# FrankVeenstra/gym_rem2D

Hardware: AMD Instinct MI355X
Metric: env steps/sec (whole node) at 65 536 parallel creatures; 1/2/4/8-GPU scaling (higher is better)
Workload: dtype f32

## Files before the change

### gym_rem2d_amd/csrc/rem2d_vel4.h

```cpp
#ifndef REM2D_VEL4_H
#define REM2D_VEL4_H

#ifndef V4_PLUS1_GAIN
#define V4_PLUS1_GAIN 2
#endif
#ifndef V4_PHASES
#ifdef REM2D_WIDE
#define V4_PHASES 5
#else
#define V4_PHASES 4
#endif
#endif
#define V4_MAX_BODIES 256
#define V4_MAX_PASSES (V4_MAX_BODIES / WAVE)

struct Vel4Args { int velIters; float dt; int prio, prioT1, prioT2;  int dbg;  };
#ifdef REM2D_V4_PROBES
#define V4_DBG(A) ((A).dbg)
#else
#define V4_DBG(A) 0

#endif

struct __attribute__((aligned(16))) V4Vel { float x, y, w, invI; };
template <int SETS, int PASSES> struct Vel4Shared {
    V4Vel vel[PASSES * WAVE];
    unsigned short jmap[SETS][WAVE];
    unsigned int cmap[PASSES * WAVE * KT];
    int firstR[PASSES * WAVE], lastR[PASSES * WAVE];
    unsigned glmap[PASSES * WAVE];
};

struct JointT {
    V2 rA, rB;
    float mA, mB;
    float exx, eyx, eyy, motorMass, det33, det22;
    float ezx, ezy, cyzx, cyzy, cyzz;
    float impX, impY, impZ, motorImp, motorSpeed, maxMotorImpulse;
    int key;
};
#define V4_JA(k) ((k) & 0xff)
#define V4_JB(k) (((k) >> 8) & 0xff)
#define V4_JROUND(k) (((k) >> 16) & 0xff)
#define V4_LIMIT(k) (((k) >> 24) & 0x3)
#define V4_JPHASE(k) (((k) >> 26) & 0x7)
#define V4_VALID(k) ((k) < 0)

DEV void v4_joint_load(const State &S, const unsigned *glmap, int K, int child, float h, int P, int rotation, JointT &J) {
    const unsigned Lp = S.Lp;
    const unsigned gl = glmap[child];
    const int jA = (child & ~(K - 1)) + LI(L_PARENT);
    const int jround = (LI(L_JROUND) & 0xff) + rotation;
    const unsigned jb = (unsigned)SCR_JREC_BASE * Lp + gl;
    J.rA = mk(SW(jb, 0), SW(jb, 1));
    J.rB = mk(SW(jb, 2), SW(jb, 3));
    J.mB = LF(L_INVM);
    const float iB = LF(L_INVI);
    J.impX = LF(L_JIMPX); J.impY = LF(L_JIMPY); J.impZ = LF(L_JIMPZ); J.motorImp = LF(L_JMOTORIMP);
    J.motorSpeed = LF(L_JMOTORSPEED);
    const int limitState = LI(L_JLIMIT);
    J.maxMotorImpulse = h * LF(L_JTORQUE);
    float iA;
    {
        const unsigned gl = glmap[jA];
        J.mA = LF(L_INVM); iA = LF(L_INVI);
    }
    J.key = jA | (child << 8) | (jround << 16) | (limitState << 24) | ((jround % P) << 26) | (int)0x80000000;
    const float mA = J.mA, mB = J.mB;
    const V2 rA = J.rA, rB = J.rB;
    J.exx = mA + mB + rA.y * rA.y * iA + rB.y * rB.y * iB;
    J.eyx = -rA.y * rA.x * iA - rB.y * rB.x * iB;
    const float ezx = -rA.y * iA - rB.y * iB;
    J.eyy = mA + mB + rA.x * rA.x * iA + rB.x * rB.x * iB;
    const float ezy = rA.x * iA + rB.x * iB;
    const float ezz = iA + iB;
    J.motorMass = iA + iB;
    if (J.motorMass > 0.0f) J.motorMass = 1.0f / J.motorMass;
    const float cyzx = J.eyy * ezz - ezy * ezy;
    const float cyzy = ezy * ezx - J.eyx * ezz;
    const float cyzz = J.eyx * ezy - J.eyy * ezx;
    J.ezx = ezx; J.ezy = ezy; J.cyzx = cyzx; J.cyzy = cyzy; J.cyzz = cyzz;
    J.det33 = J.exx * cyzx + J.eyx * cyzy + ezx * cyzz;
    if (J.det33 != 0.0f) J.det33 = 1.0f / J.det33;
    J.det22 = J.exx * J.eyy - J.eyx * J.eyx;
    if (J.det22 != 0.0f) J.det22 = 1.0f / J.det22;
}

template <typename SH> DEV void v4_joint_slot(JointT &j, SH &sh) {
    const int a = V4_JA(j.key), b = V4_JB(j.key), limitState = V4_LIMIT(j.key);
    V4Vel ra = sh.vel[a], rb = sh.vel[b];
    V2 vA = mk(ra.x, ra.y), vB = mk(rb.x, rb.y);
    float wA = ra.w, wB = rb.w;
    const float iA = ra.invI, iB = rb.invI;
    if (limitState != LIM_EQUAL) {
        float Cdot = wB - wA - j.motorSpeed;
        float impulse = -j.motorMass * Cdot;
        float oldImpulse = j.motorImp;
        j.motorImp = fclamp(oldImpulse + impulse, -j.maxMotorImpulse, j.maxMotorImpulse);
        impulse = j.motorImp - oldImpulse;
        wA -= iA * impulse;
        wB += iB * impulse;
    }
    const V2 Cdot1 = vsub(vsub(vadd(vB, vcross_sv(wB, j.rB)), vA), vcross_sv(wA, j.rA));
    float ix, iy, iz = 0.0f;
    if (limitState != LIM_INACTIVE) {
        const float ezx = j.ezx, ezy = j.ezy, ezz = iA + iB;
        const float cyzx = j.cyzx, cyzy = j.cyzy, cyzz = j.cyzz;
        float Cdot2 = wB - wA;
        float bx = Cdot1.x, by = Cdot1.y, bz = Cdot2;
        float sx = j.det33 * (bx * cyzx + by * cyzy + bz * cyzz);
        float cbx = by * ezz - bz * ezy, cby = bz * ezx - bx * ezz, cbz = bx * ezy - by * ezx;
        float sy = j.det33 * (j.exx * cbx + j.eyx * cby + ezx * cbz);
        float ebx = j.eyy * bz - ezy * by, eby = ezy * bx - j.eyx * bz, ebz = j.eyx * by - j.eyy * bx;
        float sz = j.det33 * (j.exx * ebx + j.eyx * eby + ezx * ebz);
        ix = -sx; iy = -sy; iz = -sz;
        if (limitState == LIM_EQUAL) {
            j.impX += ix; j.impY += iy; j.impZ += iz;
        } else {
            float newImpulse = j.impZ + iz;
            bool reduce = (limitState == LIM_AT_LOWER ? newImpulse : -newImpulse) < 0.0f;
            if (reduce) {
                V2 rhs = vadd(vneg(Cdot1), vscale(j.impZ, mk(ezx, ezy)));
                float rx = j.det22 * (j.eyy * rhs.x - j.eyx * rhs.y);
                float ry = j.det22 * (j.exx * rhs.y - j.eyx * rhs.x);
                ix = rx; iy = ry; iz = -j.impZ;
                j.impX += rx; j.impY += ry; j.impZ = 0.0f;
            } else {
                j.impX += ix; j.impY += iy; j.impZ += iz;
            }
        }
    } else {
        V2 bb = vneg(Cdot1);
        ix = j.det22 * (j.eyy * bb.x - j.eyx * bb.y);
        iy = j.det22 * (j.exx * bb.y - j.eyx * bb.x);
        j.impX += ix; j.impY += iy;
    }
    {
        V2 P = mk(ix, iy);
        vA = vsub(vA, vscale(j.mA, P));
        wA -= iA * (vcross(j.rA, P) + iz);
        vB = vadd(vB, vscale(j.mB, P));
        wB += iB * (vcross(j.rB, P) + iz);
    }
    ra.x = vA.x; ra.y = vA.y; ra.w = wA;
    rb.x = vB.x; rb.y = vB.y; rb.w = wB;
    sh.vel[a] = ra;
    sh.vel[b] = rb;
}

struct ContactT {
    ContactC c;
    QuadRole r;
    float mB;
    int key;
};
#define V4_CBODY(k) ((k) & 0xff)
#define V4_CSUB(k) (((k) >> 8) & 0xf)
#define V4_CT(k) (((k) >> 12) & 0xf)
static_assert(KT <= 16, "manifold index: 4 bits");
#define V4_COFF(k) (((k) >> 16) & 0xff)
#define V4_CPHASE(k) (((k) >> 24) & 0x7)

template <int CSETS, bool CPAIR, typename SH>
DEV void v4_contact_subslots(const State &S, ContactT (&C)[CSETS], SH &sh, int lane, int NC, bool spill,
                             bool pair, int nsub, int ph, int tick, int span, float mu) {
    const unsigned Lp = S.Lp;
    for (int t = 0; t < nsub; ++t) {
#pragma unroll
        for (int cs = 0; cs < CSETS; ++cs) {
            if (V4_VALID(C[cs].key) && V4_CSUB(C[cs].key) == t && V4_CPHASE(C[cs].key) == ph &&
                (unsigned)(tick - V4_COFF(C[cs].key)) < (unsigned)span) {
                const int b = V4_CBODY(C[cs].key);
                V4Vel v = sh.vel[b];
                if (!CPAIR || !pair) {
                    contact_solve(C[cs].c, C[cs].mB, v.invI, mu, v.x, v.y, v.w);
                    sh.vel[b] = v;
                } else {
                    float vq = C[cs].r.isY ? v.y : v.x;
                    contact_solve_pair(C[cs].c, C[cs].r, C[cs].mB, v.invI, mu, vq, v.w);
                    if (!C[cs].r.isY) sh.vel[b].x = vq;
                    else { sh.vel[b].y = vq; sh.vel[b].w = v.w; }
                }
            }
        }
        if (spill) {
            for (int ci = CSETS * WAVE + lane; ci < NC; ci += WAVE) {
                const int e = (int)sh.cmap[ci];
                const int b = V4_CBODY(e);
                if (V4_CSUB(e) != t || V4_CPHASE(e) != ph || !((unsigned)(tick - V4_COFF(e)) < (unsigned)span)) continue;
                const unsigned gl = sh.glmap[b];
                const unsigned cb = (unsigned)(SCR_CC_BASE + V4_CT(e) * CC_WORDS) * Lp + gl;
                ContactC c;
                cc_load(S, cb, c);
                V4Vel v = sh.vel[b];
                contact_solve(c, LF(L_INVM), v.invI, mu, v.x, v.y, v.w);
                sh.vel[b] = v;
                SW(cb, 10) = c.n0; SW(cb, 11) = c.n1; SW(cb, 12) = c.t0; SW(cb, 13) = c.t1;
            }
        }
        lds_sync();
    }
}

template <int SETS, int PASSES, int CSETS, bool CPAIR, bool FLEXP = true>
DEV void vel4_body(const State &S, const float friction, const Vel4Args &A, unsigned tile, int K, Vel4Shared<SETS, PASSES> &sh) {
    const int lane = threadIdx.x;
    const unsigned Lp = S.Lp;
    constexpr bool FLEX = FLEXP && SETS <= 3;
    const int c0 = S.tiles[tile], c1 = S.tiles[tile + 1];
    const int NB = (c1 - c0) * K;
    const unsigned long long rEntry = (V4_DBG(A) & (16 | 64)) ? __builtin_amdgcn_s_memrealtime() : 0;
    const bool retile = FLEX && (S.flags & (REM2D_FLAG_RETILE | REM2D_STATE_ORDERED)) != 0;
    const int iters = A.velIters;
    const float h = A.dt, mu = friction;
    const unsigned long long below = lane == 0 ? 0ull : (~0ull >> (WAVE - lane));
    if (S.flags & REM2D_FLAG_SKIP_FROZEN) {
        bool allSkipped = true;
        for (int e = c0 + lane; e < c1; e += WAVE) {
            const unsigned env = retile ? (unsigned)S.order[e] : (unsigned)e;
            const int m0 = __float_as_int(SW((unsigned)SCR_MISC_BASE * Lp + env * (unsigned)K, 0));
            allSkipped = allSkipped && (m0 & 0x200) != 0;
        }
        if (__all(allSkipped ? 1 : 0)) return;
    }

#pragma unroll
    for (int s = 0; s < SETS; ++s) sh.jmap[s][lane] = 0xffff;
    int sched[PASSES], misc[PASSES], parent[PASSES];
    int P = 1;
#pragma unroll
    for (int p = 0; p < PASSES; ++p) {
        const int bl = p * WAVE + lane;
        const unsigned ce = (unsigned)c0 + (unsigned)(bl / K);
        const unsigned gl = ((retile && bl < NB) ? (unsigned)S.order[ce] : ce) * (unsigned)K + (unsigned)(bl & (K - 1));
        sh.glmap[bl] = gl;
        sched[p] = 0; misc[p] = 0; parent[p] = -1;
        sh.firstR[bl] = 0x7fffffff;
        sh.lastR[bl] = -1;
        if (bl < NB) {
            misc[p] = __float_as_int(SW((unsigned)SCR_MISC_BASE * Lp + gl, 0));
            sched[p] = LI(L_JROUND);
            parent[p] = LI(L_PARENT);
            V4Vel v;
            v.x = LF(L_VX); v.y = LF(L_VY); v.w = LF(L_W); v.invI = LF(L_INVI);
            sh.vel[bl] = v;
        }
        P = max(P, (sched[p] >> 16) & 0xff);
    }
    P = wave_max(P);
    lds_sync();
#pragma unroll
    for (int p = 0; p < PASSES; ++p) {
        const int bl = p * WAVE + lane;
        if ((misc[p] & 0x100) != 0 && parent[p] >= 0) {
            const int jr = sched[p] & 0xff, pl = (bl & ~(K - 1)) + parent[p];
            atomicMin(&sh.firstR[bl], jr); atomicMax(&sh.lastR[bl], jr);
            atomicMin(&sh.firstR[pl], jr); atomicMax(&sh.lastR[pl], jr);
        }
    }
    lds_sync();
    const unsigned long long groupLanes = (K >= WAVE ? ~0ull : ((1ull << K) - 1ull)) << (lane & ~(K - 1) & (WAVE - 1));
    int offB[PASSES], delta[PASSES];
    auto plan = [&](const int Pc) -> int {
        int wlo[PASSES], wlen[PASSES];
        bool placed[PASSES];
#pragma unroll
        for (int p = 0; p < PASSES; ++p) {
            const int bl = p * WAVE + lane;
            const bool solve = (misc[p] & 0x100) != 0;
            const int nT = solve ? (misc[p] & 0xff) : 0;
            const int lastB = sh.lastR[bl];
            wlo[p] = lastB >= 0 ? lastB : 0;
            wlen[p] = lastB >= 0 ? sh.firstR[bl] + Pc - lastB : Pc;
            offB[p] = wlo[p];
            placed[p] = nT == 0;
            delta[p] = 0;
        }
        int subs[V4_PHASES];
#pragma unroll
        for (int s = 0; s < V4_PHASES; ++s) subs[s] = 0;
#pragma unroll
        for (int p = 0; p < PASSES; ++p) {
            const int wl = wlo[p] % Pc;
            for (int round = 0; round < Pc && round < V4_PHASES; ++round) {
                int cover[V4_PHASES];
#pragma unroll
                for (int s = 0; s < V4_PHASES; ++s) {
                    int d = s - wl;
                    d = d < 0 ? d + Pc : d;
                    cover[s] = __popcll(__ballot(!placed[p] && s < Pc && d < wlen[p]) & groupLanes);
                }
                int cstar = 0;
#pragma unroll
                for (int s = 1; s < V4_PHASES; ++s) cstar = (s < Pc && cover[s] >= cover[cstar]) ? s : cstar;
                int dstar = cstar - wl;
                dstar = dstar < 0 ? dstar + Pc : dstar;
                if (!placed[p] && cover[cstar] > 0 && dstar < wlen[p]) {
                    offB[p] = wlo[p] + dstar;
                    placed[p] = true;
                }
            }
            const bool solve = (misc[p] & 0x100) != 0;
            const int nT = solve ? (misc[p] & 0xff) : 0;
            if (FLEX) {
                const int cph = offB[p] % Pc;
                int heavyPhase = 0, heavy = 0;
#pragma unroll
                for (int s = 0; s < V4_PHASES; ++s) {
                    int most = 0;
#pragma unroll
                    for (int n = 1; n <= KT; ++n) most = (__ballot(nT >= n && cph == s) & groupLanes) ? n : most;
                    if (s < Pc && most > heavy) { heavy = most; heavyPhase = s; }
                }
                delta[p] = heavy > 0 ? (Pc - heavyPhase) % Pc : 0;
            }
            const int cphr = (offB[p] + delta[p]) % Pc;
#pragma unroll
            for (int s = 0; s < V4_PHASES; ++s) {
#pragma unroll
                for (int n = 1; n <= KT; ++n)
                    if (__ballot(nT >= n && cphr == s)) subs[s] = max(subs[s], n);
            }
        }
        int total = 0;
#pragma unroll
        for (int s = 0; s < V4_PHASES; ++s) total += subs[s];
        return total;
    };
    {
        const int subsP = plan(P);
        if (FLEX && P < V4_PHASES && subsP >= 3) {
            int offP[PASSES], deltaP[PASSES];
#pragma unroll
            for (int p = 0; p < PASSES; ++p) { offP[p] = offB[p]; deltaP[p] = delta[p]; }
            const int subsQ = plan(P + 1);
            if (subsQ + V4_PLUS1_GAIN <= subsP) P = P + 1;
            else {
#pragma unroll
                for (int p = 0; p < PASSES; ++p) { offB[p] = offP[p]; delta[p] = deltaP[p]; }
            }
        }
    }
#pragma unroll
    for (int p = 0; p < PASSES; ++p) sh.firstR[p * WAVE + lane] = delta[p];
    lds_sync();

    int NC = 0, lastTick = -1, maxRound = -1, err = 0, maxT = 0;
    int jcount[SETS];
#pragma unroll
    for (int s = 0; s < SETS; ++s) jcount[s] = 0;
    int subMax[V4_PHASES];
#pragma unroll
    for (int s = 0; s < V4_PHASES; ++s) subMax[s] = 0;
#pragma unroll
    for (int p = 0; p < PASSES; ++p) {
        const int bl = p * WAVE + lane;
        const bool solve = (misc[p] & 0x100) != 0;
        const bool hasJ = solve && parent[p] >= 0;
        const int nT = solve ? (misc[p] & 0xff) : 0;
        const int jr = (sched[p] & 0xff) + delta[p];
        const int phase = jr % P;
        if (!FLEX) {
#pragma unroll
            for (int s = 0; s < SETS; ++s) {
                const unsigned long long m = __ballot(hasJ && phase % SETS == s);
                if (hasJ && phase % SETS == s) {
                    const int rank = jcount[s] + __popcll(m & below);
                    if (rank < WAVE) sh.jmap[s][rank] = (unsigned short)bl;
                    else err = REM2D_ERR_SOLVER_OVERFLOW;
                }
                jcount[s] += __popcll(m);
            }
        } else {
            bool placedJ = !hasJ;
#pragma unroll
            for (int k = 0; k < SETS; ++k) {
#pragma unroll
                for (int s = 0; s < SETS; ++s) {
                    const bool want = !placedJ && (phase + k) % SETS == s;
                    const unsigned long long m = __ballot(want);
                    if (want) {
                        const int rank = jcount[s] + __popcll(m & below);
                        if (rank < WAVE) { sh.jmap[s][rank] = (unsigned short)bl; placedJ = true; }
                    }
                    jcount[s] = min(WAVE, jcount[s] + __popcll(m));
                }
            }
            if (!placedJ) err = REM2D_ERR_SOLVER_OVERFLOW;
        }
        if (hasJ && phase >= V4_PHASES) err = REM2D_ERR_SOLVER_OVERFLOW;
        const int off = offB[p] + delta[p];
        const int cph = off % P;
        if (nT > 0) {
#pragma unroll
            for (int s = 0; s < V4_PHASES; ++s)
                if (cph == s) subMax[s] = max(subMax[s], nT);
            if (cph >= V4_PHASES) err = REM2D_ERR_SOLVER_OVERFLOW;
            if (iters > 0) lastTick = max(lastTick, off + (iters - 1) * P);
        }
#pragma unroll
        for (int t = 0; t < KT; ++t) {
            const unsigned long long cm = __ballot(nT > t);
            if (nT > t) sh.cmap[NC + __popcll(cm & below)] = (unsigned)(bl | (t << 8) | (t << 12) | (off << 16) | (cph << 24));
            NC += __popcll(cm);
        }
        maxT = max(maxT, nT);
        if (iters > 0 && hasJ) lastTick = max(lastTick, jr + (iters - 1) * P);
        if (hasJ) maxRound = max(maxRound, jr);
    }
    const int nTicks = wave_max(lastTick) + 1;
    const int nRounds = wave_max(maxRound) + 1;
    maxT = wave_max(maxT);
#pragma unroll
    for (int s = 0; s < V4_PHASES; ++s) subMax[s] = (V4_DBG(A) & 1) ? 0 : wave_max(subMax[s]);
    lds_sync();
    if (A.prio & 1) {
        int cost = 7 * P;
#pragma unroll
        for (int s = 0; s < V4_PHASES; ++s) cost += 10 * subMax[s];
        if (cost >= A.prioT2) __builtin_amdgcn_s_setprio(3);
        else if (cost >= A.prioT1) __builtin_amdgcn_s_setprio(1);
    }

    JointT J[SETS];
#pragma unroll
    for (int s = 0; s < SETS; ++s) {
        J[s].key = 0;
        const int child = sh.jmap[s][lane];
        if (child != 0xffff) v4_joint_load(S, sh.glmap, K, child, h, P, sh.firstR[child], J[s]);
    }
    ContactT C[CSETS];
    const bool pair = CPAIR && NC <= CSETS * (WAVE / 2);
#pragma unroll
    for (int cs = 0; cs < CSETS; ++cs) {
        C[cs].key = 0;
        C[cs].c.count = 0;
        C[cs].mB = 0.0f;
        C[cs].r.tq = C[cs].r.nq = C[cs].r.r0c = C[cs].r.r1c = 0.0f;
        C[cs].r.isY = (lane & 1) != 0;
        C[cs].r.pt1 = false;
        const int ci = pair ? cs * (WAVE / 2) + (lane >> 1) : cs * WAVE + lane;
        if (ci < NC) {
            const int e = (int)sh.cmap[ci];
            const int b = V4_CBODY(e), t = V4_CT(e);
            const unsigned gl = sh.glmap[b];
            C[cs].key = e | (int)0x80000000;
            C[cs].mB = LF(L_INVM);
            cc_load(S, (unsigned)(SCR_CC_BASE + t * CC_WORDS) * Lp + gl, C[cs].c);
            C[cs].r = quad_role(C[cs].c, lane);
        }
    }
    const int CCAP = CSETS * WAVE;
    const bool spill = NC > CCAP;
    for (int t = 0; t < maxT; ++t) {
#pragma unroll
        for (int cs = 0; cs < CSETS; ++cs) {
            if (V4_VALID(C[cs].key) && V4_CT(C[cs].key) == t) {
                const int b = V4_CBODY(C[cs].key);
                V4Vel v = sh.vel[b];
                contact_warm_start(C[cs].c, C[cs].mB, v.invI, v.x, v.y, v.w);
                sh.vel[b] = v;
            }
        }
        if (spill) {
            for (int ci = CCAP + lane; ci < NC; ci += WAVE) {
                const int e = (int)sh.cmap[ci];
                const int b = V4_CBODY(e);
                if (V4_CT(e) != t) continue;
                const unsigned gl = sh.glmap[b];
                ContactC c;
                cc_load(S, (unsigned)(SCR_CC_BASE + t * CC_WORDS) * Lp + gl, c);
                V4Vel v = sh.vel[b];
                contact_warm_start(c, LF(L_INVM), v.invI, v.x, v.y, v.w);
                sh.vel[b] = v;
            }
        }
        lds_sync();
    }
    for (int r = 0; r < nRounds; ++r) {
#pragma unroll
        for (int s = 0; s < SETS; ++s) {
            if (V4_VALID(J[s].key) && V4_JROUND(J[s].key) == r) {
                const int a = V4_JA(J[s].key), b = V4_JB(J[s].key);
                V4Vel ra = sh.vel[a], rb = sh.vel[b];
                V2 vA = mk(ra.x, ra.y), vB = mk(rb.x, rb.y);
                float wA = ra.w, wB = rb.w;
                V2 Pw = mk(J[s].impX, J[s].impY);
                vA = vsub(vA, vscale(J[s].mA, Pw));
                wA -= ra.invI * (vcross(J[s].rA, Pw) + J[s].motorImp + J[s].impZ);
                vB = vadd(vB, vscale(J[s].mB, Pw));
                wB += rb.invI * (vcross(J[s].rB, Pw) + J[s].motorImp + J[s].impZ);
                ra.x = vA.x; ra.y = vA.y; ra.w = wA;
                rb.x = vB.x; rb.y = vB.y; rb.w = wB;
                sh.vel[a] = ra;
                sh.vel[b] = rb;
            }
        }
        lds_sync();
    }
    {
        const int span = iters * P;
        const bool joints = !(V4_DBG(A) & 2);
        const bool stamp = (V4_DBG(A) & (8 | 32)) != 0;
        unsigned long long tJ = 0, tC = 0, t0 = 0, t1 = 0, nSub = 0;
        const unsigned long long tStart = stamp ? __builtin_amdgcn_s_memtime() : 0;
        const unsigned long long rStart = stamp ? __builtin_amdgcn_s_memrealtime() : 0;
        for (int base = 0; base < nTicks; base += P) {
#pragma unroll
            for (int s = 0; s < V4_PHASES; ++s) {
                if (s < P) {
                    const int tick = base + s;
                    if (stamp) t0 = __builtin_amdgcn_s_memtime();
                    {
                        JointT &Js = J[s % SETS];
                        if (joints && V4_VALID(Js.key) && (SETS == V4_PHASES || V4_JPHASE(Js.key) == s) &&
                            (unsigned)(tick - V4_JROUND(Js.key)) < (unsigned)span) v4_joint_slot(Js, sh);
                    }
                    if (FLEX && SETS > 1) {
#pragma unroll
                        for (int q = 1; q < SETS; ++q) {
                            JointT &Jo = J[(s + q) % SETS];
                            if (joints && V4_VALID(Jo.key) && V4_JPHASE(Jo.key) == s &&
                                (unsigned)(tick - V4_JROUND(Jo.key)) < (unsigned)span) v4_joint_slot(Jo, sh);
                        }
                    }
                    lds_sync();
                    if (stamp) { t1 = __builtin_amdgcn_s_memtime(); tJ += t1 - t0; }
                    v4_contact_subslots<CSETS, CPAIR>(S, C, sh, lane, NC, spill, pair, subMax[s], s, tick, span, mu);
                    if (stamp) { tC += __builtin_amdgcn_s_memtime() - t1; nSub += subMax[s]; }
                }
            }
        }
        if ((V4_DBG(A) & 32) && lane == 0 && c1 - c0 >= 4) {
            const unsigned long long tAll = __builtin_amdgcn_s_memtime() - tStart;
            unsigned env = (unsigned)c0;
            EI(E_TOIEVENTS) = (int)(tJ >> 6);
            env = (unsigned)c0 + 1; EI(E_TOIEVENTS) = (int)(tC >> 6);
            env = (unsigned)c0 + 2; EI(E_TOIEVENTS) = (int)(tAll >> 6);
            env = (unsigned)c0 + 3; EI(E_TOIEVENTS) = (int)((nSub << 16) | (unsigned long long)(nTicks & 0xffff));
        }
        if ((V4_DBG(A) & 8) && lane == 0 && c1 - c0 >= 5) {
            const unsigned long long tAll = __builtin_amdgcn_s_memtime() - tStart;
            unsigned env = (unsigned)c0;
            EI(E_TOIEVENTS) = (int)(tJ >> 4);
            env = (unsigned)c0 + 1; EI(E_TOIEVENTS) = (int)(tC >> 4);
            env = (unsigned)c0 + 2; EI(E_TOIEVENTS) = (int)(tAll >> 4);
            env = (unsigned)c0 + 3; EI(E_TOIEVENTS) = (int)nSub;
            env = (unsigned)c0 + 4; EI(E_TOIEVENTS) = nTicks;
            if (c1 - c0 >= 6) { env = (unsigned)c0 + 5; EI(E_TOIEVENTS) = (int)(__builtin_amdgcn_s_memrealtime() - rStart); }
        }
    }
#pragma unroll
    for (int cs = 0; cs < CSETS; ++cs) {
        if (V4_VALID(C[cs].key) && !(pair && (lane & 1))) {
            const int b = V4_CBODY(C[cs].key), t = V4_CT(C[cs].key);
            const unsigned gl = sh.glmap[b];
            const slotpack_t sp = sp_load(S, (unsigned)SCR_MISC_BASE * Lp + gl);
            const unsigned o = SP_GET(sp, t) * Lp + gl;
            CF(C_N0, o) = C[cs].c.n0;
            CF(C_T0, o) = C[cs].c.t0;
            if (C[cs].c.count > 1) {
                CF(C_N1, o) = C[cs].c.n1;
                CF(C_T1, o) = C[cs].c.t1;
            }
        }
    }
    if (spill) {
        for (int ci = CCAP + lane; ci < NC; ci += WAVE) {
            const int e = (int)sh.cmap[ci];
            const int b = V4_CBODY(e), t = V4_CT(e);
            const unsigned gl = sh.glmap[b];
            const unsigned cb = (unsigned)(SCR_CC_BASE + t * CC_WORDS) * Lp + gl;
            const slotpack_t sp = sp_load(S, (unsigned)SCR_MISC_BASE * Lp + gl);
            const unsigned o = SP_GET(sp, t) * Lp + gl;
            CF(C_N0, o) = SW(cb, 10);
            CF(C_T0, o) = SW(cb, 12);
            if (__float_as_int(SW(cb, 20)) > 1) {
                CF(C_N1, o) = SW(cb, 11);
                CF(C_T1, o) = SW(cb, 13);
            }
        }
    }
#pragma unroll
    for (int s = 0; s < SETS; ++s) {
        if (V4_VALID(J[s].key)) {
            const unsigned gl = sh.glmap[V4_JB(J[s].key)];
            LF(L_JIMPX) = J[s].impX; LF(L_JIMPY) = J[s].impY; LF(L_JIMPZ) = J[s].impZ; LF(L_JMOTORIMP) = J[s].motorImp;
        }
    }
#pragma unroll
    for (int p = 0; p < PASSES; ++p) {
        const int bl = p * WAVE + lane;
        if (misc[p] & 0x100) {
            const unsigned gl = sh.glmap[bl];
            const V4Vel v = sh.vel[bl];
            LF(L_VX) = v.x; LF(L_VY) = v.y; LF(L_W) = v.w;
        }
    }
    err = wave_or(err);
    if (err) {
        for (int e = c0 + lane; e < c1; e += WAVE) {
            const unsigned env = retile ? (unsigned)S.order[e] : (unsigned)e;
            atomicOr(&EI(E_ERR), err);
        }
    }
    if ((V4_DBG(A) & 64) && lane == 0) {
        const unsigned env = (unsigned)c0;
        EI(E_TOIEVENTS) = (int)(__builtin_amdgcn_s_memrealtime() - rEntry);
    }
    if ((V4_DBG(A) & 16) && lane == 0 && c1 - c0 >= 2) {
        unsigned env = (unsigned)c0;
        EI(E_TOIEVENTS) = (int)(rEntry & 0x7fffffff);
        env = (unsigned)c0 + 1; EI(E_TOIEVENTS) = (int)(__builtin_amdgcn_s_memrealtime() & 0x7fffffff);
    }
}

struct Vel4Batch {
    State S[REM2D_MAX_BATCH];
    float friction[REM2D_MAX_BATCH];
    unsigned tileEnd[REM2D_MAX_BATCH];
    int lanes[REM2D_MAX_BATCH];
    int n;
};
template <int SETS, int PASSES, int CSETS, int WPS, bool CPAIR, bool FLEXP = true>
__global__ __launch_bounds__(WAVE, WPS) void rem2d_vel4_kernel(Vel4Batch B, Vel4Args A) {
    __shared__ Vel4Shared<SETS, PASSES> sh;
    unsigned tile = blockIdx.x;
    int b = 0;
    while (b + 1 < B.n && tile >= B.tileEnd[b]) ++b;
    if (b > 0) tile -= B.tileEnd[b - 1];
    vel4_body<SETS, PASSES, CSETS, CPAIR, FLEXP>(B.S[b], B.friction[b], A, tile, B.lanes[b], sh);
}

struct VelPostShared {
    union {
        Vel4Shared<1, 1> v;
        PosShared p;
    };
};
#ifndef REM2D_VELPOST_WAVES
#define REM2D_VELPOST_WAVES 1
#endif
__global__ __launch_bounds__(WAVE * REM2D_VELPOST_WAVES, 4) void rem2d_velpost_kernel(Batch B, StepArgs A, Vel4Args V) {
    __shared__ VelPostShared sh;
    if (REM2D_VELPOST_WAVES > 1 && threadIdx.x >= WAVE) return;
    unsigned block = blockIdx.x;
    const int b = batch_find(B, block);
    {
        const int K = B.lanes[b];
        const unsigned cpb = (unsigned)(WAVE / K), cap = (unsigned)B.S[b].tileCap;
        const unsigned t1 = (block + 1) * cpb / cap;
        for (unsigned t = block * cpb / cap; t < t1 && t < (unsigned)B.S[b].nTiles; ++t) {
            vel4_body<1, 1, 1, true>(B.S[b], B.T[b].friction, V, t, K, sh.v);
            lds_sync();
        }
    }
    __builtin_amdgcn_fence(__ATOMIC_RELEASE, "workgroup");
    __builtin_amdgcn_fence(__ATOMIC_ACQUIRE, "workgroup");
    BATCH_DISPATCH(post_only_body, sh.p)
}

template <int K> DEV void pre_intile_body(const State &S, const Terrain &T, const StepArgs &A, unsigned block) { pre_body<K, true>(S, T, A, block); }
template <int K>
DEV void post_toi_body(const State &S, const Terrain &T, const StepArgs &A, unsigned block, PosShared &psh, ToiSharedT<1> &ts1, int bad) {
    const bool heavy = post_body<K, true>(S, T, A, block, psh);
    const int lane = threadIdx.x;
    const unsigned slot = (block * WAVE + lane) / K;
    const unsigned env = (S.flags & REM2D_STATE_ORDERED) ? (unsigned)S.order[slot] : slot;
    if (bad && (lane & (K - 1)) == 0) EI(E_ERR) = EI(E_ERR) | REM2D_ERR_HANDOVER;
    if (A.defer != 2) return;
    const unsigned mygl = env * K + (unsigned)(lane & (K - 1));
    __builtin_amdgcn_fence(__ATOMIC_RELEASE, "workgroup");
    __builtin_amdgcn_fence(__ATOMIC_ACQUIRE, "workgroup");
    unsigned long long hm = __ballot(heavy ? 1 : 0);
#ifdef REM2D_PROBE_SKIP_TOI
    hm = 0ull;
#endif
    while (hm) {
        const int h = __ffsll((long long)hm) - 1;
        hm &= hm - 1;
        const unsigned glh = (unsigned)__shfl((int)mygl, h);
        toi_heavy_one<K, 1>(S, T, A, glh, ts1, lane, WAVE);
        __builtin_amdgcn_fence(__ATOMIC_RELEASE, "workgroup");
        __builtin_amdgcn_fence(__ATOMIC_ACQUIRE, "workgroup");
    }
}
#define TRAIN_FLAG_WORDS 16
#define TRAIN_STEP_BITS 28
#define TRAIN_STEP_MASK ((1u << TRAIN_STEP_BITS) - 1u)
#define TRAIN_WAIT_TICKS 200000000ull
#define TRAIN_FAULT_DROP (1 << 30)
DEV bool train_fault_hits(int fault, int step, unsigned blk) {
    const int s = fault & 0xffff;
    const unsigned m = (unsigned)((fault >> 16) & 0x3fff);
    return fault != 0 && step == s && (m <= 1u || blk % m == 0u);
}
DEV int train_acquire(unsigned *flags, unsigned fl, int step, unsigned xcd, int fault, unsigned blk, unsigned *failures) {
    int bad = 0;
    if (threadIdx.x == 0) {
        const unsigned long long t0 = __builtin_amdgcn_s_memrealtime();
        unsigned seen;
        while (((seen = __hip_atomic_load(&flags[fl], __ATOMIC_RELAXED, __HIP_MEMORY_SCOPE_AGENT)) & TRAIN_STEP_MASK) < (unsigned)step) {
            __builtin_amdgcn_s_sleep(32);
            if (__hip_atomic_load(&flags[1], __ATOMIC_RELAXED, __HIP_MEMORY_SCOPE_AGENT) != 0u) { bad = 1; break; }
            if (__builtin_amdgcn_s_memrealtime() - t0 > TRAIN_WAIT_TICKS) {
                __hip_atomic_store(&flags[1], 1u, __ATOMIC_RELAXED, __HIP_MEMORY_SCOPE_AGENT);
                bad = 1;
                break;
            }
        }
        if ((seen >> TRAIN_STEP_BITS) != xcd) bad = 1;
        if (!(fault & TRAIN_FAULT_DROP) && train_fault_hits(fault, step, blk)) bad = 1;
        if (bad) __hip_atomic_fetch_add(failures, 1u, __ATOMIC_RELAXED, __HIP_MEMORY_SCOPE_SYSTEM);
    }
    bad = __builtin_amdgcn_readfirstlane(bad);
    asm volatile("buffer_inv sc1\n\ts_dcache_inv\n\ts_waitcnt vmcnt(0) lgkmcnt(0)" ::: "memory");
    return bad;
}
DEV void train_release(unsigned *flags, unsigned fl, int step, unsigned xcd, int fault, unsigned blk) {
    asm volatile("s_waitcnt vmcnt(0) lgkmcnt(0)" ::: "memory");
    if (threadIdx.x == 0 && !((fault & TRAIN_FAULT_DROP) && train_fault_hits(fault, step + 1, blk)))
        __hip_atomic_store(&flags[fl], (unsigned)(step + 1) | (xcd << TRAIN_STEP_BITS), __ATOMIC_RELAXED, __HIP_MEMORY_SCOPE_AGENT);
}
#define TRAIN_XCC_ID() ((unsigned)__builtin_amdgcn_s_getreg((3 << 11) | (0 << 6) | 20) & 15u)

__global__ __launch_bounds__(WAVE, 4) void rem2d_step_train_kernel(Batch B, StepArgs A, Vel4Args V, unsigned *flags, unsigned nBlocks, int fault,
                                                                    unsigned *failures) {
    __shared__ VelPostShared sh;
    __shared__ ToiSharedT<1> ts1;
    const unsigned nPad = (nBlocks + 7u) & ~7u;
    const unsigned item = blockIdx.x;
    const int step = (int)(item / nPad);
    const unsigned slot = item % nPad;
    if (slot >= nBlocks) return;
    const unsigned blk = nBlocks - 1 - slot;
    const unsigned xcd = TRAIN_XCC_ID();
    int bad = 0;
    if (step > 0) bad = train_acquire(flags, TRAIN_FLAG_WORDS + blk, step, xcd, fault, blk, failures);
    unsigned block = blk;
    const int b = batch_find(B, block);
    BATCH_DISPATCH(pre_intile_body)
    __builtin_amdgcn_fence(__ATOMIC_RELEASE, "workgroup");
    __builtin_amdgcn_fence(__ATOMIC_ACQUIRE, "workgroup");
    {
        const int K = B.lanes[b];
        const unsigned cpb = (unsigned)(WAVE / K), cap = (unsigned)B.S[b].tileCap;
        const unsigned t1 = (block + 1) * cpb / cap;
        for (unsigned t = block * cpb / cap; t < t1 && t < (unsigned)B.S[b].nTiles; ++t) {
            vel4_body<1, 1, 1, true>(B.S[b], B.T[b].friction, V, t, K, sh.v);
            lds_sync();
        }
    }
    __builtin_amdgcn_fence(__ATOMIC_RELEASE, "workgroup");
    __builtin_amdgcn_fence(__ATOMIC_ACQUIRE, "workgroup");
    BATCH_DISPATCH(post_toi_body, sh.p, ts1, bad)
    train_release(flags, TRAIN_FLAG_WORDS + blk, step, xcd, fault, blk);
}

struct Train128Shared {
    union {
        Vel4Shared<2, 2> v;
        PosShared p;
    };
};
template <bool FLEXP, int WPS>
__global__ __launch_bounds__(WAVE, WPS) void rem2d_step_train128_kernel(Batch B, StepArgs A, Vel4Args V, unsigned *flags, unsigned nItems, int fault,
                                                                         unsigned *failures) {
    __shared__ Train128Shared sh;
    __shared__ ToiSharedT<1> ts1;
    const unsigned nPad = (nItems + 7u) & ~7u;
    const unsigned item = blockIdx.x;
    const int step = (int)(item / nPad);
    const unsigned slot = item % nPad;
    if (slot >= nItems) return;
    const unsigned idx = nItems - 1 - slot;
    unsigned it = idx;
    int b = 0;
    unsigned bpt = 1, blocksW = 0;
    for (;; ++b) {
        blocksW = B.blockEnd[b] - (b ? B.blockEnd[b - 1] : 0u);
        const unsigned lanesPerTile = (unsigned)B.S[b].tileCap * (unsigned)B.lanes[b];
        bpt = lanesPerTile > WAVE ? lanesPerTile / WAVE : 1u;
        const unsigned itemsW = (blocksW + bpt - 1) / bpt;
        if (it < itemsW || b + 1 >= B.n) break;
        it -= itemsW;
    }
    const unsigned blk0 = it * bpt, nb = blk0 + bpt <= blocksW ? bpt : blocksW - blk0;
    const unsigned xcd = TRAIN_XCC_ID();
    int bad = 0;
    if (step > 0) bad = train_acquire(flags, TRAIN_FLAG_WORDS + idx, step, xcd, fault, idx, failures);
    for (unsigned p = 0; p < nb; ++p) {
        unsigned block = blk0 + p;
        BATCH_DISPATCH(pre_intile_body)
    }
    __builtin_amdgcn_fence(__ATOMIC_RELEASE, "workgroup");
    __builtin_amdgcn_fence(__ATOMIC_ACQUIRE, "workgroup");
    {
        const int K = B.lanes[b];
        const unsigned cpb = (unsigned)(WAVE / K), cap = (unsigned)B.S[b].tileCap;
        const bool whole = cap * (unsigned)K > WAVE;
        const unsigned ta = whole ? it : blk0 * cpb / cap, tb = whole ? it + 1 : (blk0 + 1) * cpb / cap;
        for (unsigned t = ta; t < tb && t < (unsigned)B.S[b].nTiles; ++t) {
            vel4_body<2, 2, 1, false, FLEXP>(B.S[b], B.T[b].friction, V, t, K, sh.v);
            lds_sync();
        }
    }
    __builtin_amdgcn_fence(__ATOMIC_RELEASE, "workgroup");
    __builtin_amdgcn_fence(__ATOMIC_ACQUIRE, "workgroup");
    for (unsigned p = 0; p < nb; ++p) {
        unsigned block = blk0 + p;
        BATCH_DISPATCH(post_toi_body, sh.p, ts1, bad)
        lds_sync();
    }
    train_release(flags, TRAIN_FLAG_WORDS + idx, step, xcd, fault, idx);
}

#endif
```

Before: 72.12 million.

## Add steady-state tick loop with precomputed slot codes for joints and contacts

Adds a steady-state path for the velocity solver. It applies to the window of ticks in which every joint and contact is already active and none has finished its iterations. Inside that window the per-tick round/offset range checks are dropped, and slot membership is precomputed as small phase/subslot codes. Cross-set joint slots that no lane uses anywhere in the wave are skipped through a ballot mask. The spill path is specialised at compile time, so the inner loops carry less per-slot predicate and key-decoding work, at the cost of more code size and register pressure.

```diff
diff --git a/gym_rem2d_amd/csrc/rem2d_vel4.h b/gym_rem2d_amd/csrc/rem2d_vel4.h
--- a/gym_rem2d_amd/csrc/rem2d_vel4.h
+++ b/gym_rem2d_amd/csrc/rem2d_vel4.h
@@ -10,6 +10,9 @@
 #else
 #define V4_PHASES 4
 #endif
+#endif
+#ifndef V4_STEADY
+#define V4_STEADY 1
 #endif
 #define V4_MAX_BODIES 256
 #define V4_MAX_PASSES (V4_MAX_BODIES / WAVE)
@@ -161,41 +164,67 @@
 #define V4_COFF(k) (((k) >> 16) & 0xff)
 #define V4_CPHASE(k) (((k) >> 24) & 0x7)
 
+template <bool CPAIR, typename SH> DEV void v4_contact_lane(ContactT &c, SH &sh, bool pair, float mu) {
+    const int b = V4_CBODY(c.key);
+    V4Vel v = sh.vel[b];
+    if (!CPAIR || !pair) {
+        contact_solve(c.c, c.mB, v.invI, mu, v.x, v.y, v.w);
+        sh.vel[b] = v;
+    } else {
+        float vq = c.r.isY ? v.y : v.x;
+        contact_solve_pair(c.c, c.r, c.mB, v.invI, mu, vq, v.w);
+        if (!c.r.isY) sh.vel[b].x = vq;
+        else { sh.vel[b].y = vq; sh.vel[b].w = v.w; }
+    }
+}
+
+template <typename SH> DEV void v4_contact_spilled(const State &S, SH &sh, int e, float mu) {
+    const unsigned Lp = S.Lp;
+    const int b = V4_CBODY(e);
+    const unsigned gl = sh.glmap[b];
+    const unsigned cb = (unsigned)(SCR_CC_BASE + V4_CT(e) * CC_WORDS) * Lp + gl;
+    ContactC c;
+    cc_load(S, cb, c);
+    V4Vel v = sh.vel[b];
+    contact_solve(c, LF(L_INVM), v.invI, mu, v.x, v.y, v.w);
+    sh.vel[b] = v;
+    SW(cb, 10) = c.n0; SW(cb, 11) = c.n1; SW(cb, 12) = c.t0; SW(cb, 13) = c.t1;
+}
+
 template <int CSETS, bool CPAIR, typename SH>
 DEV void v4_contact_subslots(const State &S, ContactT (&C)[CSETS], SH &sh, int lane, int NC, bool spill,
                              bool pair, int nsub, int ph, int tick, int span, float mu) {
-    const unsigned Lp = S.Lp;
     for (int t = 0; t < nsub; ++t) {
 #pragma unroll
         for (int cs = 0; cs < CSETS; ++cs) {
             if (V4_VALID(C[cs].key) && V4_CSUB(C[cs].key) == t && V4_CPHASE(C[cs].key) == ph &&
-                (unsigned)(tick - V4_COFF(C[cs].key)) < (unsigned)span) {
-                const int b = V4_CBODY(C[cs].key);
-                V4Vel v = sh.vel[b];
-                if (!CPAIR || !pair) {
-                    contact_solve(C[cs].c, C[cs].mB, v.invI, mu, v.x, v.y, v.w);
-                    sh.vel[b] = v;
-                } else {
-                    float vq = C[cs].r.isY ? v.y : v.x;
-                    contact_solve_pair(C[cs].c, C[cs].r, C[cs].mB, v.invI, mu, vq, v.w);
-                    if (!C[cs].r.isY) sh.vel[b].x = vq;
-                    else { sh.vel[b].y = vq; sh.vel[b].w = v.w; }
-                }
-            }
+                (unsigned)(tick - V4_COFF(C[cs].key)) < (unsigned)span) v4_contact_lane<CPAIR>(C[cs], sh, pair, mu);
         }
         if (spill) {
             for (int ci = CSETS * WAVE + lane; ci < NC; ci += WAVE) {
                 const int e = (int)sh.cmap[ci];
-                const int b = V4_CBODY(e);
                 if (V4_CSUB(e) != t || V4_CPHASE(e) != ph || !((unsigned)(tick - V4_COFF(e)) < (unsigned)span)) continue;
-                const unsigned gl = sh.glmap[b];
-                const unsigned cb = (unsigned)(SCR_CC_BASE + V4_CT(e) * CC_WORDS) * Lp + gl;
-                ContactC c;
-                cc_load(S, cb, c);
-                V4Vel v = sh.vel[b];
-                contact_solve(c, LF(L_INVM), v.invI, mu, v.x, v.y, v.w);
-                sh.vel[b] = v;
-                SW(cb, 10) = c.n0; SW(cb, 11) = c.n1; SW(cb, 12) = c.t0; SW(cb, 13) = c.t1;
+                v4_contact_spilled(S, sh, e, mu);
+            }
+        }
+        lds_sync();
+    }
+}
+
+#define V4_CCODE(ph, t) (((ph) << 4) | (t))
+template <bool B> struct V4Bool { static constexpr bool value = B; };
+template <int CSETS, bool CPAIR, bool SPILL, typename SH>
+DEV void v4_contact_subslots_steady(const State &S, ContactT (&C)[CSETS], const int (&ccode)[CSETS], SH &sh, int lane, int NC,
+                                    bool pair, int nsub, int ph, float mu) {
+    for (int t = 0; t < nsub; ++t) {
+#pragma unroll
+        for (int cs = 0; cs < CSETS; ++cs)
+            if (ccode[cs] == V4_CCODE(ph, t)) v4_contact_lane<CPAIR>(C[cs], sh, pair, mu);
+        if (SPILL) {
+            for (int ci = CSETS * WAVE + lane; ci < NC; ci += WAVE) {
+                const int e = (int)sh.cmap[ci];
+                if (V4_CSUB(e) != t || V4_CPHASE(e) != ph) continue;
+                v4_contact_spilled(S, sh, e, mu);
             }
         }
         lds_sync();
@@ -346,6 +375,7 @@
     lds_sync();
 
     int NC = 0, lastTick = -1, maxRound = -1, err = 0, maxT = 0;
+    int firstHi = 0, firstLo = 0x7fffff;
     int jcount[SETS];
 #pragma unroll
     for (int s = 0; s < SETS; ++s) jcount[s] = 0;
@@ -397,6 +427,7 @@
                 if (cph == s) subMax[s] = max(subMax[s], nT);
             if (cph >= V4_PHASES) err = REM2D_ERR_SOLVER_OVERFLOW;
             if (iters > 0) lastTick = max(lastTick, off + (iters - 1) * P);
+            firstHi = max(firstHi, off); firstLo = min(firstLo, off);
         }
 #pragma unroll
         for (int t = 0; t < KT; ++t) {
@@ -406,10 +437,11 @@
         }
         maxT = max(maxT, nT);
         if (iters > 0 && hasJ) lastTick = max(lastTick, jr + (iters - 1) * P);
-        if (hasJ) maxRound = max(maxRound, jr);
+        if (hasJ) { maxRound = max(maxRound, jr); firstHi = max(firstHi, jr); firstLo = min(firstLo, jr); }
     }
     const int nTicks = wave_max(lastTick) + 1;
     const int nRounds = wave_max(maxRound) + 1;
+    const int tLo = wave_max(firstHi), tHi = -wave_max(-firstLo) + iters * P;
     maxT = wave_max(maxT);
 #pragma unroll
     for (int s = 0; s < V4_PHASES; ++s) subMax[s] = (V4_DBG(A) & 1) ? 0 : wave_max(subMax[s]);
@@ -505,7 +537,58 @@
         unsigned long long tJ = 0, tC = 0, t0 = 0, t1 = 0, nSub = 0;
         const unsigned long long tStart = stamp ? __builtin_amdgcn_s_memtime() : 0;
         const unsigned long long rStart = stamp ? __builtin_amdgcn_s_memrealtime() : 0;
-        for (int base = 0; base < nTicks; base += P) {
+        const bool steadyOK = V4_STEADY && joints && !stamp && tLo < tHi;
+        int jcode[SETS], ccode[CSETS];
+        unsigned jlook = 0;
+#pragma unroll
+        for (int q = 0; q < SETS; ++q) jcode[q] = -1;
+#pragma unroll
+        for (int cs = 0; cs < CSETS; ++cs) ccode[cs] = -1;
+        if (steadyOK) {
+#pragma unroll
+            for (int q = 0; q < SETS; ++q)
+                jcode[q] = !V4_VALID(J[q].key) ? -1 : SETS == V4_PHASES ? q : V4_JPHASE(J[q].key);
+#pragma unroll
+            for (int cs = 0; cs < CSETS; ++cs)
+                ccode[cs] = V4_VALID(C[cs].key) ? V4_CCODE(V4_CPHASE(C[cs].key), V4_CSUB(C[cs].key)) : -1;
+#pragma unroll
+            for (int s = 0; s < V4_PHASES; ++s) {
+#pragma unroll
+                for (int q = 1; q < ((FLEX && SETS > 1) ? SETS : 1); ++q)
+                    if (__ballot(jcode[(s + q) % SETS] == s)) jlook |= 1u << (q * 8 + s);
+            }
+        }
+        int base = 0;
+        auto steady_groups = [&](auto withSpill) {
+                for (; base + P <= tHi; base += P) {
+#pragma unroll
+                    for (int s = 0; s < V4_PHASES; ++s) {
+                        if (s < P) {
+                            {
+                                JointT &Js = J[s % SETS];
+                                if (jcode[s % SETS] == s) v4_joint_slot(Js, sh);
+                            }
+                            if (FLEX && SETS > 1) {
+#pragma unroll
+                                for (int q = 1; q < SETS; ++q) {
+                                    if (jlook & (1u << (q * 8 + s))) {
+                                        JointT &Jo = J[(s + q) % SETS];
+                                        if (jcode[(s + q) % SETS] == s) v4_joint_slot(Jo, sh);
+                                    }
+                                }
+                            }
+                            lds_sync();
+                            v4_contact_subslots_steady<CSETS, CPAIR, decltype(withSpill)::value>(S, C, ccode, sh, lane, NC, pair, subMax[s], s, mu);
+                        }
+                    }
+                }
+        };
+        for (; base < nTicks; base += P) {
+            if (steadyOK && base >= tLo) {
+                if (spill) steady_groups(V4Bool<true>());
+                else steady_groups(V4Bool<false>());
+                if (base >= nTicks) break;
+            }
 #pragma unroll
             for (int s = 0; s < V4_PHASES; ++s) {
                 if (s < P) {
```

Measured after the change: 74.12 million (median of 6 runs). 1.03x the previous value.
